# 1275468127/Medical-SAM2

Hardware: AMD Instinct MI355X
Metric: slices/sec @1024^2 (Hiera-S) (higher is better)
Workload: dtype bf16; 1 GPU; configs[1]: sam2_hiera_s 2D (train_2d SAM2 sub-sequence, forward), b=4 x 1024x1024 per GPU, 16-entry memory bank with 4 sampled memories per slice, one click per slice; forward_image -> memory_attention -> prompt encoder -> mask decoder -> memory encoder; hip_graph=True, weights=random name-keyed init

## Files before the change

### include/msam2_hip.h

```cpp
#ifndef MSAM2_HIP_H
#define MSAM2_HIP_H

#include <stddef.h>
#include <stdint.h>

#ifdef __cplusplus
extern "C" {
#endif

const char* msam2_last_error(void);

int msam2_version(void);

int msam2_operand_is_fp16(void);

int msam2_graph_begin(void* stream);

int msam2_graph_end(void* stream, void** graph_exec_out);

int msam2_graph_launch(void* graph_exec, void* stream);

int msam2_graph_destroy(void* graph_exec);

int msam2_event_create(void** ev);

int msam2_event_record(void* ev, void* stream);

int msam2_event_elapsed_ms(void* start, void* stop, float* ms);

int msam2_event_destroy(void* ev);

int msam2_gemm_nt(const void* A, int64_t lda, const void* B, int64_t ldb, const float* bias, const void* residual, int64_t ldr, void* C, int64_t ldc, int out_is_16bit, int64_t M, int64_t N, int64_t K, void* stream);

int msam2_gemm(const void* A, int64_t lda, const void* W, int64_t ldw, const float* bias, const float* colscale, const void* residual, int64_t ldr, int res_is_16bit, int64_t res_mod, void* C, int64_t ldc, int out_is_16bit, int64_t M, int64_t N, int64_t K, int act, void* stream);

int msam2_gemm_tokens(const float* A, int64_t lda, const float* A2, int64_t add_cols, const void* W, int64_t ldw, const float* bias, const float* residual, int64_t ldr, void* C, int64_t ldc, int out_is_16bit, int64_t M, int64_t N, int64_t K, int act, void* stream);

int msam2_gemm_pool2x2(const void* A, int64_t lda, const void* W, int64_t ldw, const float* bias, float* C, int64_t ldc, int64_t B, int64_t H, int64_t Wimg, int64_t N, int64_t K, void* stream);

int msam2_gemm_qkv_pool2x2(const void* A, int64_t lda, const void* W, int64_t ldw, const float* bias, void* QKV, int64_t ldc, void* Q2, int64_t ldq, int64_t B, int64_t H, int64_t Wimg, int64_t N, int64_t K, int64_t q_cols, void* stream);

int msam2_gemm_rope(const void* A, int64_t lda, const void* W, int64_t ldw, const float* bias, void* C, int64_t ldc, int64_t M, int64_t N, int64_t K, const float* rope_cos, const float* rope_sin, int64_t rope_cols, int64_t head_dim, int64_t rows_per_batch, int64_t n_rope, int64_t n_pos, void* stream);

int msam2_gemm_residual_layernorm_supported(int64_t N, int64_t K);

int msam2_gemm_residual_layernorm(const void* A, int64_t lda, const void* W, int64_t ldw, const float* bias, const float* R32, int64_t ldr, float* C32, int64_t ldc, const float* ln_w, const float* ln_b, float eps, void* Y16, int64_t ldy, int64_t M, int64_t N, int64_t K, void* stream);

int msam2_gemm_merged_residual_layernorm_supported(int64_t N, int64_t D, int splits);

int msam2_gemm_merged_residual_layernorm(const void* workspace, size_t workspace_bytes, int splits, int64_t D, const void* W, int64_t ldw, const float* bias, const float* R32, int64_t ldr, float* C32, int64_t ldc, const float* ln_w, const float* ln_b, float eps, void* Y16, int64_t ldy, int64_t M, int64_t N, void* stream);

size_t msam2_attention_workspace_bytes(int64_t Bz, int64_t H, int64_t Lq, int64_t D, int splits);

int msam2_attention_merge(void* o, const int64_t* o_strides, int64_t B, int64_t H, int64_t Lq, int64_t Lk, int64_t D, int splits, void* workspace, size_t workspace_bytes, void* stream);

int msam2_attention_fwd(const void* q, const int64_t* q_strides, const void* k, const int64_t* k_strides, const void* v, const int64_t* v_strides, void* o, const int64_t* o_strides, int64_t B, int64_t H, int64_t Lq, int64_t Lk, int64_t D, float scale, int splits, void* workspace, size_t workspace_bytes, void* stream);

int msam2_attention_fwd_lse(const void* q, const int64_t* q_strides, const void* k, const int64_t* k_strides, const void* v, const int64_t* v_strides, void* o, const int64_t* o_strides, int64_t B, int64_t H, int64_t Lq, int64_t Lk, int64_t D, float scale, int splits, void* workspace, size_t workspace_bytes, float* lse, void* stream);

int msam2_attention_fwd_lse_dropout(const void* q, const int64_t* q_strides, const void* k, const int64_t* k_strides, const void* v, const int64_t* v_strides, void* o, const int64_t* o_strides, int64_t B, int64_t H, int64_t Lq, int64_t Lk, int64_t D, float scale, int splits, void* workspace, size_t workspace_bytes, float* lse, float p, uint64_t seed, uint64_t offset, const void* seed_dev, void* stream);

int msam2_attention_kv64_fwd(const void* q, const int64_t* q_strides, const void* k, const int64_t* k_strides, const void* v, const int64_t* v_strides, void* o, const int64_t* o_strides, int64_t B, int64_t H, int64_t Lq, int64_t Lk, float scale, int splits, void* workspace, size_t workspace_bytes, void* stream);

int msam2_attention_effective_splits(int64_t Lk, int splits);

int msam2_attention_kv64_partial(const void* q, const int64_t* q_strides, const void* k, const int64_t* k_strides, const void* v, const int64_t* v_strides, int64_t B, int64_t H, int64_t Lq, int64_t Lk, float scale, int splits, int split_begin, int split_count, void* workspace, size_t workspace_bytes, void* stream);

int msam2_attention_kv64_dyn_fwd(const void* q, const int64_t* q_strides, const void* k, const int64_t* k_strides, const void* v, const int64_t* v_strides, void* o, const int64_t* o_strides, int64_t B, int64_t H, int64_t Lq, int64_t Lk, const void* key_count_dev, float scale, int splits, void* workspace, size_t workspace_bytes, void* stream);

int msam2_attention_kv64_dyn_partial(const void* q, const int64_t* q_strides, const void* k, const int64_t* k_strides, const void* v, const int64_t* v_strides, int64_t B, int64_t H, int64_t Lq, int64_t Lk, const void* key_count_dev, float scale, int splits, int split_begin, int split_count, void* workspace, size_t workspace_bytes, void* stream);

int msam2_window_attention_fwd(const void* q, int64_t q_token_stride, int64_t q_head_stride, int64_t hq, int64_t wq, int64_t ws_q, const void* k, const void* v, int64_t kv_token_stride, int64_t kv_head_stride, int64_t hk, int64_t wk, int64_t ws_k, const float* kpad, const float* vpad, void* o, int64_t o_token_stride, int64_t o_head_stride, int64_t B, int64_t H, int64_t D, float scale, void* stream);

int msam2_attention_small_fwd(const void* q, int64_t q_bs, int64_t q_ts, const void* k, int64_t k_bs, int64_t k_ts, const void* v, int64_t v_bs, int64_t v_ts, void* o, int64_t o_bs, int64_t o_ts, int64_t B, int64_t H, int64_t Lq, int64_t Lk, int64_t D, float scale, void* stream);

int msam2_attention_fewq_keysplit_splits(int64_t B, int64_t H);

int msam2_attention_fewq_keysplit(const void* q, int64_t q_bs, int64_t q_ts, const void* k, int64_t k_bs, int64_t k_ts, const void* v, int64_t v_bs, int64_t v_ts, float* part, int64_t B, int64_t H, int64_t Lq, int64_t Lk, int64_t D, int64_t splits, float scale, void* stream);

int msam2_window_qkv_attention_supported(int64_t dim, int64_t dim_out, int64_t heads, int64_t ws, int pool, int64_t H, int64_t W);

int msam2_window_qkv_attention_fwd(const void* xn, const void* w, const float* bias, void* o, int64_t B, int64_t H, int64_t W, int64_t dim, int64_t heads, int64_t ws, int pool, float scale, void* stream);

// ... 241 lines not shown
```

### medical-sam2_amd/_lib.py

```python
from __future__ import annotations

import ctypes
import os
import subprocess

_HERE = os.path.dirname(os.path.abspath(__file__))
LIB_PATH = os.environ.get("MSAM2_LIB_PATH") or os.path.join(_HERE, "libmsam2_hip.so")

c_p = ctypes.c_void_p
c_i = ctypes.c_int
c_l = ctypes.c_int64
c_f = ctypes.c_float
c_z = ctypes.c_size_t
c_d = ctypes.c_double

SIGNATURES = {
    "msam2_version": (c_i, []),
    "msam2_last_error": (ctypes.c_char_p, []),
    "msam2_operand_is_fp16": (c_i, []),
    "msam2_gemm": (c_i, [c_p, c_l, c_p, c_l, c_p, c_p, c_p, c_l, c_i, c_l, c_p, c_l, c_i, c_l, c_l, c_l, c_i, c_p]),
    "msam2_gemm_pool2x2": (c_i, [c_p, c_l, c_p, c_l, c_p, c_p, c_l, c_l, c_l, c_l, c_l, c_l, c_p]),
    "msam2_gemm_qkv_pool2x2": (c_i, [c_p, c_l, c_p, c_l, c_p, c_p, c_l, c_p, c_l, c_l, c_l, c_l, c_l, c_l, c_l, c_p]),
    "msam2_gemm_tokens": (c_i, [c_p, c_l, c_p, c_l, c_p, c_l, c_p, c_p, c_l, c_p, c_l, c_i, c_l, c_l, c_l, c_i, c_p]),
    "msam2_gemm_rope": (c_i, [c_p, c_l, c_p, c_l, c_p, c_p, c_l, c_l, c_l, c_l, c_p, c_p, c_l, c_l, c_l, c_l, c_l, c_p]),
    "msam2_gemm_residual_layernorm_supported": (c_i, [c_l, c_l]),
    "msam2_gemm_residual_layernorm": (c_i, [c_p, c_l, c_p, c_l, c_p, c_p, c_l, c_p, c_l, c_p, c_p, c_f, c_p, c_l, c_l, c_l, c_l, c_p]),
    "msam2_gemm_merged_residual_layernorm_supported": (c_i, [c_l, c_l, c_i]),
    "msam2_gemm_merged_residual_layernorm": (c_i, [c_p, c_z, c_i, c_l, c_p, c_l, c_p, c_p, c_l, c_p, c_l, c_p, c_p, c_f, c_p, c_l, c_l, c_l, c_p]),
    "msam2_ln_mlp_residual_supported": (c_i, [c_l]),
    "msam2_mlp_fused_permute_w2": (c_i, [c_p, c_p, c_l, c_l, c_p]),
    "msam2_ln_mlp_residual_fwd": (c_i, [c_p, c_l, c_l, c_p, c_p, c_f, c_p, c_p, c_p, c_p, c_p, c_p]),
    "msam2_ln_mlp_residual_fwd_dual": (c_i, [c_p, c_l, c_l, c_p, c_p, c_f, c_p, c_p, c_p, c_p, c_p, c_p, c_p]),
    "msam2_proj_ln_mlp_residual_supported": (c_i, [c_l]),
    "msam2_mlp_fused_permute_w1": (c_i, [c_p, c_p, c_l, c_l, c_p]),
    "msam2_proj_ln_mlp_residual_fwd": (c_i, [c_p, c_p, c_p, c_p, c_l, c_l, c_p, c_p, c_f, c_p, c_p, c_p, c_p, c_p, c_p, c_p, c_p, c_f, c_p, c_p]),
    "msam2_layernorm": (c_i, [c_p, c_i, c_l, c_p, c_p, c_p, c_i, c_l, c_l, c_l, c_f, c_i, c_p]),
    "msam2_layernorm_dual": (c_i, [c_p, c_l, c_p, c_p, c_p, c_l, c_p, c_l, c_l, c_l, c_f, c_p]),
    "msam2_attention_workspace_bytes": (c_z, [c_l, c_l, c_l, c_l, c_i]),
    "msam2_attention_fwd": (c_i, [c_p, c_p, c_p, c_p, c_p, c_p, c_p, c_p, c_l, c_l, c_l, c_l, c_l, c_f, c_i, c_p, c_z, c_p]),
    "msam2_attention_fwd_lse": (c_i, [c_p, c_p, c_p, c_p, c_p, c_p, c_p, c_p, c_l, c_l, c_l, c_l, c_l, c_f, c_i, c_p, c_z, c_p, c_p]),
    "msam2_attention_fwd_lse_dropout": (c_i, [c_p, c_p, c_p, c_p, c_p, c_p, c_p, c_p, c_l, c_l, c_l, c_l, c_l, c_f, c_i, c_p, c_z, c_p, c_f,
                                              ctypes.c_uint64, ctypes.c_uint64, c_p, c_p]),
    "msam2_attention_kv64_fwd": (c_i, [c_p, c_p, c_p, c_p, c_p, c_p, c_p, c_p, c_l, c_l, c_l, c_l, c_f, c_i, c_p, c_z, c_p]),
    "msam2_attention_kv64_partial": (c_i, [c_p, c_p, c_p, c_p, c_p, c_p, c_l, c_l, c_l, c_l, c_f, c_i, c_i, c_i, c_p, c_z, c_p]),
    "msam2_attention_kv64_dyn_fwd": (c_i, [c_p, c_p, c_p, c_p, c_p, c_p, c_p, c_p, c_l, c_l, c_l, c_l, c_p, c_f, c_i, c_p, c_z, c_p]),
    "msam2_attention_kv64_dyn_partial": (c_i, [c_p, c_p, c_p, c_p, c_p, c_p, c_l, c_l, c_l, c_l, c_p, c_f, c_i, c_i, c_i, c_p, c_z, c_p]),
    "msam2_attention_effective_splits": (c_i, [c_l, c_i]),
    "msam2_attention_merge": (c_i, [c_p, c_p, c_l, c_l, c_l, c_l, c_l, c_i, c_p, c_z, c_p]),
    "msam2_window_attention_fwd": (c_i, [c_p, c_l, c_l, c_l, c_l, c_l, c_p, c_p, c_l, c_l, c_l, c_l, c_l, c_p, c_p, c_p, c_l, c_l,
                                         c_l, c_l, c_l, c_f, c_p]),
    "msam2_window_qkv_attention_supported": (c_i, [c_l, c_l, c_l, c_l, c_i, c_l, c_l]),
    "msam2_window_qkv_attention_fwd": (c_i, [c_p, c_p, c_p, c_p, c_l, c_l, c_l, c_l, c_l, c_l, c_i, c_f, c_p]),
    "msam2_attention_small_fwd": (c_i, [c_p, c_l, c_l, c_p, c_l, c_l, c_p, c_l, c_l, c_p, c_l, c_l, c_l, c_l, c_l, c_l, c_l, c_f,
                                        c_p]),
    "msam2_add_cast": (c_i, [c_p, c_i, c_l, c_l, c_p, c_i, c_l, c_l, c_f, c_p, c_i, c_l, c_l, c_l, c_p]),
    "msam2_maxpool2x2": (c_i, [c_p, c_i, c_l, c_p, c_i, c_l, c_l, c_l, c_l, c_l, c_p]),
    "msam2_upsample2x_add": (c_i, [c_p, c_p, c_l, c_l, c_l, c_l, c_p]),
    "msam2_rope_table": (c_i, [c_p, c_p, c_l, c_l, c_f, c_p]),
    "msam2_rope_inplace": (c_i, [c_p, c_l, c_l, c_l, c_l, c_l, c_l, c_l, c_p, c_p, c_p]),
    "msam2_bilinear_upsample": (c_i, [c_p, c_p, c_l, c_l, c_l, c_l, c_l, c_p]),
    "msam2_sine_pos_2d": (c_i, [c_p, c_l, c_l, c_l, c_f, c_p]),
# ... 154 lines not shown
```

### medical-sam2_amd/modeling/encoder.py

```python
from __future__ import annotations

from typing import List, Optional, Tuple

import torch
import torch.nn as nn

from .. import ops
from .common import OP16, F32, WeightCache, nchw_view, to_bf16, tokens_of, v_f32, w_bf16
from .position import PositionEmbeddingSine


import os as _os
_POOL_GEMM = _os.environ.get("MSAM2_NO_POOL_GEMM") is None
_QPOOL_GEMM = _os.environ.get("MSAM2_NO_QPOOL_GEMM") is None
_FUSED_MLP = _os.environ.get("MSAM2_NO_FUSED_MLP") is None
_FUSED_QKV_ATTN = _os.environ.get("MSAM2_NO_FUSED_QKV_ATTN") is None
_FUSED_PATCH = _os.environ.get("MSAM2_NO_FUSED_PATCH") is None
_FUSED_GEMM_LN = _os.environ.get("MSAM2_NO_FUSED_GEMM_LN") is None
_FUSED_GEMM_LN_K = frozenset(int(k) for k in _os.environ.get("MSAM2_FUSED_GEMM_LN_K", "384,1536").split(",") if k.strip())
_FUSED_PROJ_MLP = _os.environ.get("MSAM2_NO_FUSED_PROJ_MLP") is None
_FUSED_PROJ_MLP_DIMS = frozenset(int(k) for k in _os.environ.get("MSAM2_FUSED_PROJ_MLP_DIMS", "96,192").split(",") if k.strip())
_FUSED_PROJ_MLP_NEXT_LN_DIMS = frozenset(int(k) for k in _os.environ.get("MSAM2_FUSED_PROJ_MLP_NEXT_LN_DIMS", "").split(",") if k.strip())
_TWO_LAUNCH = 0


class two_launch_qkv_attention:

    def __enter__(self):
        global _TWO_LAUNCH
        _TWO_LAUNCH += 1

    def __exit__(self, *exc):
        global _TWO_LAUNCH
        _TWO_LAUNCH -= 1
        return False


def _gemm_ln_dispatched(N: int, K: int) -> bool:
    return _FUSED_GEMM_LN and K in _FUSED_GEMM_LN_K and ops.gemm_residual_layernorm_supported(N, K)


def _proj_mlp_dispatched(dim_out: int, width: int) -> bool:
    return _FUSED_PROJ_MLP and width == dim_out and dim_out in _FUSED_PROJ_MLP_DIMS and ops.proj_ln_mlp_residual_supported(dim_out)


def frozen_forward_image(model, imgs: torch.Tensor) -> dict:
    with two_launch_qkv_attention():
        return model.forward_image(imgs)


class PatchEmbed(nn.Module):

    def __init__(self, kernel_size=(7, 7), stride=(4, 4), padding=(3, 3), in_chans: int = 3, embed_dim: int = 768):
        super().__init__()
        assert tuple(kernel_size) == (7, 7) and tuple(stride) == (4, 4) and tuple(padding) == (3, 3) and in_chans == 3, \
            "the HIP path implements the 7x7/4/3 RGB patch embedding used by every SAM2 config"
        self.proj = nn.Conv2d(in_chans, embed_dim, kernel_size=kernel_size, stride=stride, padding=padding)
        self._wc = WeightCache()

    def _weight(self):
        def build():
            w = torch.zeros(self.proj.weight.shape[0], 160, dtype=OP16, device=self.proj.weight.device)
            w[:, :147] = self.proj.weight.detach().reshape(-1, 147).to(OP16)
            return w
        return self._wc.get("w", [self.proj.weight], build)

    def _weight_perm(self):
        def build():
            w = self.proj.weight.detach()
            E = w.shape[0]
            wp = torch.zeros((E + 31) // 32 * 32, 22, 8, dtype=OP16, device=w.device)
            wp[:E, :21, 1:] = w.reshape(E, 21, 7).to(OP16)
            return wp.reshape(-1, 176).contiguous()
        return self._wc.get("wp", [self.proj.weight], build)

    def tokens(self, x: torch.Tensor, pos: Optional[torch.Tensor] = None) -> torch.Tensor:
        x = x.to(F32).contiguous()
        E = self.proj.weight.shape[0]
        if _FUSED_PATCH and ops.patch_embed_supported(x.shape[-1], E) and x.shape[-1] == x.shape[-2] and (pos is None or pos.shape[0] == (x.shape[-1] // 4) ** 2):
            return ops.patch_embed(x, self._weight_perm(), v_f32(self._wc, "b", self.proj.bias), None if pos is None else pos.to(F32).contiguous())
        cols = ops.im2col_patch(x)
        return ops.gemm(cols, self._weight(), v_f32(self._wc, "b", self.proj.bias), residual=pos,
                        res_mod=pos.shape[0] if pos is not None else 0, out_dtype=F32)

    def forward(self, x: torch.Tensor) -> torch.Tensor:
        B, _, S, _ = x.shape
        return self.tokens(x).reshape(B, S // 4, S // 4, -1)


class MLP(nn.Module):

    def __init__(self, input_dim: int, hidden_dim: int, output_dim: int, num_layers: int, activation: nn.Module = nn.ReLU,
                 sigmoid_output: bool = False):
        super().__init__()
        self.num_layers = num_layers
        h = [hidden_dim] * (num_layers - 1)
        self.layers = nn.ModuleList(nn.Linear(n, k) for n, k in zip([input_dim] + h, h + [output_dim]))
        self.sigmoid_output = sigmoid_output
        self.act = activation()
        self._act_code = ops.ACT_GELU if isinstance(self.act, nn.GELU) else ops.ACT_RELU
        self._wc = WeightCache()

    def run(self, x_bf16: torch.Tensor, residual: Optional[torch.Tensor] = None, out_dtype=F32, ln=None):
        h = x_bf16
        for i, layer in enumerate(self.layers):
            last = i == self.num_layers - 1
            last_act = ops.ACT_SIGMOID if self.sigmoid_output else ops.ACT_NONE
            if (last and ln is not None and residual is not None and out_dtype == F32 and last_act == ops.ACT_NONE
                    and _gemm_ln_dispatched(layer.out_features, layer.in_features)):
                return ops.gemm_residual_layernorm(h, w_bf16(self._wc, f"w{i}", layer.weight), v_f32(self._wc, f"b{i}", layer.bias), residual, *ln)
            h = ops.gemm(h, w_bf16(self._wc, f"w{i}", layer.weight), v_f32(self._wc, f"b{i}", layer.bias),
                         act=last_act if last else self._act_code, residual=residual if last else None,
                         out_dtype=out_dtype if last else OP16)
        return h if ln is None else (h, None)

    def run_tokens(self, x: torch.Tensor) -> torch.Tensor:
        L = self.layers
        if (self.num_layers == 3 and self._act_code == ops.ACT_RELU and x.shape[0] <= 4096 and L[0].in_features == 256
                and L[0].out_features == 256 and L[1].out_features == 256 and L[2].out_features <= 256):
            def pack():
                dev = x.device
                n = L[2].out_features
                w3 = torch.zeros(1, 256, 256, dtype=OP16, device=dev)
                b3 = torch.zeros(1, 256, dtype=F32, device=dev)
                w3[0, :n] = L[2].weight.detach().to(OP16)
                b3[0, :n] = L[2].bias.detach().float()
                return (L[0].weight.detach().to(OP16)[None].contiguous(), L[0].bias.detach().float()[None].contiguous(),
                        L[1].weight.detach().to(OP16)[None].contiguous(), L[1].bias.detach().float()[None].contiguous(), w3, b3)

            def consts():
                dev = x.device
                return (torch.zeros(1, dtype=torch.int32, device=dev), torch.tensor([L[2].out_features], dtype=torch.int32, device=dev),
                        torch.tensor([int(self.sigmoid_output)], dtype=torch.int32, device=dev))
            tok, od, sg = self._wc.get("tok3_const", [], consts)
            w1, b1, w2, b2, w3, b3 = self._wc.get("tok3", [t for l in L for t in (l.weight, l.bias)], pack)
            y = ops.token_mlp3(x.to(F32).contiguous().view(x.shape[0], 1, 256), tok, w1, b1, w2, b2, w3, b3, od, sg)
            return y[:, 0, : L[2].out_features].contiguous()
# ... 98 lines not shown
                q = (qp.view(B, Hq * Wq, heads, Dp) if pool else v5[:, :, 0]).permute(0, 2, 1, 3)
                o = ops.attention(q, v5[:, :, 1].permute(0, 2, 1, 3), v5[:, :, 2].permute(0, 2, 1, 3), scale=scale)
                o = o.permute(0, 2, 1, 3).reshape(B * Hq * Wq, width)
        mlp = self.mlp
        one_kernel_mlp = (_FUSED_MLP and ops.ln_mlp_residual_supported(dim_out) and mlp.num_layers == 2 and mlp._act_code == ops.ACT_GELU
                          and mlp.layers[0].out_features == 4 * dim_out and Hq * Wq >= 1024)
        if fused_gemm_ln and attn_in_one_kernel and one_kernel_mlp and _proj_mlp_dispatched(dim_out, width):
            w1p = mlp._wc.get("w0p", [mlp.layers[0].weight], lambda: ops.mlp_fused_permute_w1(mlp.layers[0].weight.detach().to(OP16).contiguous()))
            w2p = mlp._wc.get("w1p", [mlp.layers[1].weight], lambda: ops.mlp_fused_permute_w2(mlp.layers[1].weight.detach().to(OP16).contiguous()))
            next_ln = next_norm if next_norm is not None and dim_out in _FUSED_PROJ_MLP_NEXT_LN_DIMS else None
            t, out16, self.next_xn = ops.proj_ln_mlp_residual(o, proj_w, v_f32(wc, "ob", a.proj.bias), shortcut, v_f32(wc, "n2w", self.norm2.weight),
                                                              v_f32(wc, "n2b", self.norm2.bias), 1e-6, w1p, v_f32(mlp._wc, "b0", mlp.layers[0].bias),
                                                              w2p, v_f32(mlp._wc, "b1", mlp.layers[1].bias), also16=emit16, next_ln=next_ln)
            if emit16:
                self.out16 = out16
            return t, Hq, Wq
        xn2 = None
        if fused_gemm_ln and not one_kernel_mlp and _gemm_ln_dispatched(dim_out, width):
            t, xn2 = ops.gemm_residual_layernorm(o, proj_w, v_f32(wc, "ob", a.proj.bias), shortcut,
                                                 v_f32(wc, "n2w", self.norm2.weight), v_f32(wc, "n2b", self.norm2.bias), 1e-6)
        else:
            t = ops.gemm(o, proj_w, v_f32(wc, "ob", a.proj.bias), residual=shortcut, out_dtype=F32)
        if one_kernel_mlp:
            w2p = mlp._wc.get("w1p", [mlp.layers[1].weight], lambda: ops.mlp_fused_permute_w2(mlp.layers[1].weight.detach().to(OP16).contiguous()))
            t = ops.ln_mlp_residual(t, v_f32(wc, "n2w", self.norm2.weight), v_f32(wc, "n2b", self.norm2.bias), 1e-6,
                                    w_bf16(mlp._wc, "w0", mlp.layers[0].weight), v_f32(mlp._wc, "b0", mlp.layers[0].bias), w2p,
                                    v_f32(mlp._wc, "b1", mlp.layers[1].bias), also16=emit16)
            if emit16:
                t, self.out16 = t
            return t, Hq, Wq
        if xn2 is None:
            xn2 = ops.layernorm(t, v_f32(wc, "n2w", self.norm2.weight), v_f32(wc, "n2b", self.norm2.bias), 1e-6)
        if fused_gemm_ln and next_norm is not None:
            t, self.next_xn = mlp.run(xn2, residual=t, out_dtype=F32, ln=next_norm)
        else:
            t = mlp.run(xn2, residual=t, out_dtype=F32)
        return t, Hq, Wq

    def forward(self, x: torch.Tensor) -> torch.Tensor:
        B, H, W, C = x.shape
        t, h, w = self.run(x.to(F32).reshape(B * H * W, C).contiguous(), B, H, W)
        return t.reshape(B, h, w, -1)


class Hiera(nn.Module):

    def __init__(self, embed_dim: int = 96, num_heads: int = 1, drop_path_rate: float = 0.0, q_pool: int = 3,
                 q_stride: Tuple[int, int] = (2, 2), stages: Tuple[int, ...] = (2, 3, 16, 3), dim_mul: float = 2.0,
                 head_mul: float = 2.0, window_pos_embed_bkg_spatial_size: Tuple[int, int] = (14, 14),
                 window_spec: Tuple[int, ...] = (8, 4, 14, 7), global_att_blocks: Tuple[int, ...] = (12, 16, 20),
                 return_interm_layers=True):
        super().__init__()
        assert len(stages) == len(window_spec) and drop_path_rate == 0.0
        self.window_spec = window_spec
        depth = sum(stages)
        self.q_stride = q_stride
        self.stage_ends = [sum(stages[:i]) - 1 for i in range(1, len(stages) + 1)]
        self.q_pool_blocks = [x + 1 for x in self.stage_ends[:-1]][:q_pool]
        self.return_interm_layers = return_interm_layers
        self.patch_embed = PatchEmbed(embed_dim=embed_dim)
        self.global_att_blocks = global_att_blocks
        self.window_pos_embed_bkg_spatial_size = window_pos_embed_bkg_spatial_size
        self.pos_embed = nn.Parameter(torch.zeros(1, embed_dim, *window_pos_embed_bkg_spatial_size))
        self.pos_embed_window = nn.Parameter(torch.zeros(1, embed_dim, window_spec[0], window_spec[0]))
        cur_stage = 1
        self.blocks = nn.ModuleList()
        for i in range(depth):
# ... 111 lines not shown
```

### medical-sam2_amd/ops.py

```python
from __future__ import annotations

import ctypes
import math
from typing import Optional, Tuple

import torch

from ._lib import check, lib

OP16 = torch.float16 if lib().msam2_operand_is_fp16() else torch.bfloat16

F32 = torch.float32
ACT_NONE, ACT_GELU, ACT_RELU, ACT_SIGMOID = 0, 1, 2, 3


def _stream() -> int:
    return torch.cuda.current_stream().cuda_stream


def _p(t: Optional[torch.Tensor]):
    return None if t is None else t.data_ptr()


def _is_bf16(t: torch.Tensor) -> int:
# ... 195 lines not shown
    x2 = x.reshape(-1, C)
    _req(x2.dtype == F32 and x2.stride(1) == 1 and C % 4 == 0, "layernorm_dual: fp32 rows, C % 4 == 0")
    y = torch.empty(x2.shape, dtype=F32, device=x.device)
    y16 = torch.empty(x2.shape, dtype=OP16, device=x.device)
    check(lib().msam2_layernorm_dual(_p(x2), x2.stride(0), _p(weight), _p(bias), _p(y), y.stride(0), _p(y16), y16.stride(0), x2.shape[0], C, eps,
                                     _stream()))
    return y.reshape(x.shape), y16.reshape(x.shape)


def gemm_residual_layernorm_supported(N: int, K: int) -> bool:
    return bool(lib().msam2_gemm_residual_layernorm_supported(N, K))


def gemm_residual_layernorm(a: torch.Tensor, w: torch.Tensor, bias: Optional[torch.Tensor], residual: torch.Tensor, ln_w: torch.Tensor,
                            ln_b: torch.Tensor, eps: float, *, out: Optional[torch.Tensor] = None, out16: Optional[torch.Tensor] = None):
    _req(a.dim() == 2 and w.dim() == 2 and a.shape[1] == w.shape[1], f"gemm_residual_layernorm shapes {tuple(a.shape)} x {tuple(w.shape)}")
    _req(a.dtype == OP16 and w.dtype == OP16 and a.stride(1) == 1 and w.stride(1) == 1, "gemm_residual_layernorm operands: 16-bit, K-contiguous")
    M, K = a.shape
    N = w.shape[0]
    _req(gemm_residual_layernorm_supported(N, K),
         f"gemm_residual_layernorm: N = {N}, K = {K} is not built (N = 384 with K % 64 == 0; N = 256 with K = 64, 256 or 2048)")
    _req(residual.dtype == F32 and residual.shape == (M, N) and residual.stride(1) == 1, "gemm_residual_layernorm: residual must be fp32 [M, N]")
    _req(ln_w.dtype == F32 and ln_b.dtype == F32 and ln_w.numel() == N and ln_b.numel() == N and ln_w.is_contiguous() and ln_b.is_contiguous()
         and (bias is None or (bias.dtype == F32 and bias.numel() == N and bias.is_contiguous())),
         "gemm_residual_layernorm: bias, ln_w, ln_b are fp32 [N]")
    if out is None:
        out = torch.empty(M, N, dtype=F32, device=a.device)
    if out16 is None:
        out16 = torch.empty(M, N, dtype=OP16, device=a.device)
    _req(out.dtype == F32 and out.shape == (M, N) and out.stride(1) == 1 and out16.dtype == OP16 and out16.shape == (M, N) and out16.stride(1) == 1,
         "gemm_residual_layernorm: out is fp32 [M, N], out16 16-bit [M, N], rows contiguous")
    check(lib().msam2_gemm_residual_layernorm(_p(a), a.stride(0), _p(w), w.stride(0), _p(bias), _p(residual), residual.stride(0), _p(out),
                                              out.stride(0), _p(ln_w), _p(ln_b), float(eps), _p(out16), out16.stride(0), M, N, K, _stream()))
    return out, out16


def gemm_merged_residual_layernorm_supported(N: int, D: int, splits: int) -> bool:
    return bool(lib().msam2_gemm_merged_residual_layernorm_supported(N, D, splits))


def gemm_merged_residual_layernorm(workspace: torch.Tensor, splits: int, D: int, w: torch.Tensor, bias: Optional[torch.Tensor],
                                   residual: torch.Tensor, ln_w: torch.Tensor, ln_b: torch.Tensor, eps: float, *,
                                   out: Optional[torch.Tensor] = None, out16: Optional[torch.Tensor] = None):
    _req(w.dim() == 2 and w.dtype == OP16 and w.stride(1) == 1 and w.shape[1] == D, f"gemm_merged_residual_layernorm: w is 16-bit [N, {D}], K-contiguous")
    _req(workspace.dtype == torch.uint8 and workspace.is_contiguous(), "gemm_merged_residual_layernorm: workspace is a contiguous uint8 buffer")
    N = w.shape[0]
    _req(residual.dim() == 2 and residual.dtype == F32 and residual.shape[1] == N and residual.stride(1) == 1,
         "gemm_merged_residual_layernorm: residual must be fp32 [M, N]")
    M = residual.shape[0]
    _req(ln_w.dtype == F32 and ln_b.dtype == F32 and ln_w.numel() == N and ln_b.numel() == N and ln_w.is_contiguous() and ln_b.is_contiguous()
         and (bias is None or (bias.dtype == F32 and bias.numel() == N and bias.is_contiguous())),
         "gemm_merged_residual_layernorm: bias, ln_w, ln_b are fp32 [N]")
    if out is None:
        out = torch.empty(M, N, dtype=F32, device=w.device)
    if out16 is None:
        out16 = torch.empty(M, N, dtype=OP16, device=w.device)
    _req(out.dtype == F32 and out.shape == (M, N) and out.stride(1) == 1 and out16.dtype == OP16 and out16.shape == (M, N) and out16.stride(1) == 1,
         "gemm_merged_residual_layernorm: out is fp32 [M, N], out16 16-bit [M, N], rows contiguous")
    check(lib().msam2_gemm_merged_residual_layernorm(_p(workspace), workspace.numel(), int(splits), int(D), _p(w), w.stride(0), _p(bias), _p(residual),
                                                     residual.stride(0), _p(out), out.stride(0), _p(ln_w), _p(ln_b), float(eps), _p(out16),
                                                     out16.stride(0), M, N, _stream()))
    return out, out16


def ln_mlp_residual_supported(dim: int) -> bool:
    return bool(lib().msam2_ln_mlp_residual_supported(dim))
# ... 1259 lines not shown
```

Measured before the change: 754.9 slices/s.

## Fuse Hiera MLP fc1+GELU+fc2+residual+LayerNorm into one kernel for dim 384

Adds a single HIP kernel that, for each 64-row tile, computes fc1 in 128-wide hidden chunks, applies bias and GELU, keeps the hidden chunk in LDS, and accumulates fc2. It then adds the residual and writes fp32 output plus the next block's LayerNorm output. The encoder dispatches to it for 384-wide stages with at least 1024 tokens. This avoids writing the 4x-wide hidden activation to global memory and saves launches. In exchange it uses 160KB of LDS with one block per CU, and every hidden chunk runs behind serialized barriers, so the kernel may be less efficient than separate tuned GEMMs.

```diff
diff --git a/include/msam2_hip.h b/include/msam2_hip.h
--- a/include/msam2_hip.h
+++ b/include/msam2_hip.h
@@ -49,6 +49,10 @@
 int msam2_gemm_merged_residual_layernorm_supported(int64_t N, int64_t D, int splits);
 
 int msam2_gemm_merged_residual_layernorm(const void* workspace, size_t workspace_bytes, int splits, int64_t D, const void* W, int64_t ldw, const float* bias, const float* R32, int64_t ldr, float* C32, int64_t ldc, const float* ln_w, const float* ln_b, float eps, void* Y16, int64_t ldy, int64_t M, int64_t N, void* stream);
+
+int msam2_mlp_residual_layernorm_supported(int64_t N, int64_t H);
+
+int msam2_mlp_residual_layernorm_fwd(const void* A, int64_t lda, const void* W1, int64_t ldw1, const float* b1, const void* W2, int64_t ldw2, const float* b2, const float* R32, int64_t ldr, float* C32, int64_t ldc, const float* ln_w, const float* ln_b, float eps, void* Y16, int64_t ldy, int64_t M, int64_t N, int64_t H, void* stream);
 
 size_t msam2_attention_workspace_bytes(int64_t Bz, int64_t H, int64_t Lq, int64_t D, int splits);
 
diff --git a/medical-sam2_amd/_lib.py b/medical-sam2_amd/_lib.py
--- a/medical-sam2_amd/_lib.py
+++ b/medical-sam2_amd/_lib.py
@@ -27,6 +27,8 @@
     "msam2_gemm_residual_layernorm": (c_i, [c_p, c_l, c_p, c_l, c_p, c_p, c_l, c_p, c_l, c_p, c_p, c_f, c_p, c_l, c_l, c_l, c_l, c_p]),
     "msam2_gemm_merged_residual_layernorm_supported": (c_i, [c_l, c_l, c_i]),
     "msam2_gemm_merged_residual_layernorm": (c_i, [c_p, c_z, c_i, c_l, c_p, c_l, c_p, c_p, c_l, c_p, c_l, c_p, c_p, c_f, c_p, c_l, c_l, c_l, c_p]),
+    "msam2_mlp_residual_layernorm_supported": (c_i, [c_l, c_l]),
+    "msam2_mlp_residual_layernorm_fwd": (c_i, [c_p, c_l, c_p, c_l, c_p, c_p, c_l, c_p, c_p, c_l, c_p, c_l, c_p, c_p, c_f, c_p, c_l, c_l, c_l, c_l, c_p]),
     "msam2_ln_mlp_residual_supported": (c_i, [c_l]),
     "msam2_mlp_fused_permute_w2": (c_i, [c_p, c_p, c_l, c_l, c_p]),
     "msam2_ln_mlp_residual_fwd": (c_i, [c_p, c_l, c_l, c_p, c_p, c_f, c_p, c_p, c_p, c_p, c_p, c_p]),
diff --git a/medical-sam2_amd/csrc/mlp_rowln.hip b/medical-sam2_amd/csrc/mlp_rowln.hip
--- /dev/null
+++ b/medical-sam2_amd/csrc/mlp_rowln.hip
@@ -0,0 +1,344 @@
+#include "common.h"
+
+struct MlpRowLnParams {
+  const op16* A;
+  const op16* W1;
+  const op16* W2;
+  const float* b1;
+  const float* b2;
+  const float* R;
+  float* C;
+  const float* ln_w;
+  const float* ln_b;
+  op16* Y;
+  int64_t lda, ldw1, ldw2, ldr, ldc, ldy;
+  int M, H;
+  float eps;
+};
+
+template <int N, int LAD>
+__global__ __launch_bounds__(512, 1) void mlp_rowln_kernel(MlpRowLnParams p) {
+#if defined(__HIP_DEVICE_COMPILE__)
+  typedef Img128 Img;
+  constexpr int BM = 64, BK = 64, KS = BK / 16, HC = 128;
+  constexpr int KT = N / BK;
+  constexpr int A_BYTES = BM * BK * 2;
+  constexpr int RES_BYTES = KT * A_BYTES;
+  constexpr int HID_BYTES = (HC / BK) * A_BYTES;
+  constexpr int STAGE_BYTES = N * BK * 2;
+  constexpr int W1IMG_BYTES = HC * BK * 2;
+  constexpr int PPW = STAGE_BYTES / 1024 / 8;
+  constexpr int FN = N / 4 / 32;
+  constexpr int TLD = N + 4;
+  constexpr int CH = N / 64;
+  static_assert(N == 384, "one instance: the stage of 48 KB holds W1's 128 rows x 192 k as well as W2's 384 rows x 64 k");
+  static_assert((KT / 2) * W1IMG_BYTES == STAGE_BYTES && PPW * 8 * 1024 == STAGE_BYTES && BM == 8 * Img::PIECE_ROWS, "8 waves share the pieces evenly");
+  static_assert(BM * TLD * 4 <= RES_BYTES + HID_BYTES + 2 * STAGE_BYTES, "the epilogue tile aliases the images and the ring");
+  extern __shared__ __attribute__((aligned(1024))) unsigned char lds[];
+  unsigned char* const hid = lds + RES_BYTES;
+  unsigned char* const ring = hid + HID_BYTES;
+  const int tid = threadIdx.x;
+  const int wave = __builtin_amdgcn_readfirstlane(tid >> 6), lane = tid & 63;
+  const int ws = wave >> 2, wq = wave & 3;
+  const int r = lane & 31, h = lane >> 5;
+  const int64_t m0 = (int64_t)xcd_tile_order(blockIdx.x, gridDim.x) * BM;
+  if (m0 >= p.M) return;
+
+  float bias_j[FN];
+#pragma unroll
+  for (int j = 0; j < FN; ++j) bias_j[j] = p.b2 ? p.b2[wq * (N / 4) + j * 32 + r] : 0.f;
+
+  const auto a_rsrc = raw_rsrc(p.A);
+  const auto w1_rsrc = raw_rsrc(p.W1);
+  const auto w2_rsrc = raw_rsrc(p.W2);
+  unsigned offsW1[PPW], offsW2[PPW];
+#pragma unroll
+  for (int i = 0; i < PPW; ++i) {
+    const int q = wave * PPW + i;
+    const int row1 = Img::piece_row(q & 15, lane);
+    offsW1[i] = (unsigned)((int64_t)row1 * p.ldw1 * 2 + (q >> 4) * (BK * 2) + Img::src_chunk(row1, lane) * 16);
+    const int row2 = Img::piece_row(q, lane);
+    offsW2[i] = (unsigned)((int64_t)row2 * p.ldw2 * 2 + Img::src_chunk(row2, lane) * 16);
+  }
+  auto issue = [&](int c, int t) __attribute__((always_inline)) {
+    unsigned char* base = ring + (t & 1) * STAGE_BYTES + wave * (PPW * 1024);
+    if ((LAD & 8) && c > 0) return;
+    if (t < 2) {
+      const unsigned so = (unsigned)((int64_t)c * HC * p.ldw1 * 2) + (unsigned)t * (N / 2) * 2;
+#pragma unroll
+      for (int i = 0; i < PPW; ++i) glds16(w1_rsrc, base + i * 1024, offsW1[i], so);
+    } else {
+      const unsigned so = (unsigned)(c * HC + (t - 2) * BK) * 2;
+#pragma unroll
+      for (int i = 0; i < PPW; ++i) glds16(w2_rsrc, base + i * 1024, offsW2[i], so);
+    }
+  };
+
+  {
+    const int row = Img::piece_row(wave, lane);
+    const unsigned offsA = (unsigned)(min(m0 + row, (int64_t)p.M - 1) * p.lda * 2 + Img::src_chunk(row, lane) * 16);
+#pragma unroll
+    for (int i = 0; i < KT; ++i) glds16(a_rsrc, lds + i * A_BYTES + wave * 1024, offsA, (unsigned)i * BK * 2);
+  }
+  {
+    const int j = (blockIdx.x >> 3) & 31;
+    unsigned char* dst = ring + STAGE_BYTES + wave * 1024;
+    {
+      const int cpr = N >> 3, rows = p.H >> 5, n = rows * cpr;
+      for (int i = wave; i * 64 < n; i += 8) {
+        const int q = min(i * 64 + lane, n - 1);
+        const int row = j * rows + q / cpr, c = q - (q / cpr) * cpr;
+        glds16(w1_rsrc, dst, (unsigned)((int64_t)row * p.ldw1 * 2 + c * 16), 0);
+      }
+    }
+    {
+      const int cpr = p.H >> 3, n = (N / 32) * cpr;
+      for (int i = wave; i * 64 < n; i += 8) {
+        const int q = min(i * 64 + lane, n - 1);
+        const int row = j * (N / 32) + q / cpr, c = q - (q / cpr) * cpr;
+        glds16(w2_rsrc, dst, (unsigned)((int64_t)row * p.ldw2 * 2 + c * 16), 0);
+      }
+    }
+  }
+
+  f32x16 acc[FN];
+  zero_acc(acc);
+
+  const int ra = ws * 32 + r;
+  const int offA = ra * Img::ROW_BYTES, swzA = Img::swz(ra);
+  const int r1 = wq * 32 + r;
+  const int offW1 = r1 * Img::ROW_BYTES, swzW1 = Img::swz(r1);
+  int offB[FN], swzB[FN];
+#pragma unroll
+  for (int j = 0; j < FN; ++j) {
+    const int rb = wq * (N / 4) + j * 32 + r;
+    offB[j] = rb * Img::ROW_BYTES;
+    swzB[j] = Img::swz(rb);
+  }
+  unsigned char* const hdst = hid + (wq >> 1) * A_BYTES + offA + 8 * h;
+  const int hc0 = (wq & 1) * 4;
+
+  f32x16 acc1;
+  f32x4 b1v[4];
+  auto fc1_half = [&](int t) __attribute__((always_inline)) {
+    const unsigned char* sb = ring + (t & 1) * STAGE_BYTES;
+#pragma unroll
+    for (int kl = 0; kl < KT / 2; ++kl) {
+      const unsigned char* sw = sb + kl * W1IMG_BYTES;
+      const unsigned char* sx = lds + (t * (KT / 2) + kl) * A_BYTES;
+      op16x8 wf[KS], xf[KS];
+#pragma unroll
+      for (int ks = 0; ks < KS; ++ks) {
+        const int c = 2 * ks + h;
+        wf[ks] = *reinterpret_cast<const op16x8*>(sw + offW1 + ((c ^ swzW1) << 4));
+        xf[ks] = *reinterpret_cast<const op16x8*>(sx + offA + ((c ^ swzA) << 4));
+      }
+#pragma unroll
+      for (int ks = 0; ks < KS; ++ks) {
+        if constexpr (LAD & 2) acc1[ks] += op2f(wf[ks][0]) + op2f(xf[ks][0]);
+        else acc1 = MSAM2_MFMA_32x32x16(wf[ks], xf[ks], acc1, 0, 0, 0);
+      }
+    }
+  };
+  auto fc2_step = [&](int u) __attribute__((always_inline)) {
+    const unsigned char* sb = ring + u * STAGE_BYTES;
+    const unsigned char* sa = hid + u * A_BYTES;
+    op16x8 af[KS], bfr[KS][FN];
+#pragma unroll
+    for (int ks = 0; ks < KS; ++ks) {
+      const int c = 2 * ks + h;
+      af[ks] = *reinterpret_cast<const op16x8*>(sa + offA + ((c ^ swzA) << 4));
+#pragma unroll
+      for (int j = 0; j < FN; ++j) bfr[ks][j] = *reinterpret_cast<const op16x8*>(sb + offB[j] + ((c ^ swzB[j]) << 4));
+    }
+#pragma unroll
+    for (int ks = 0; ks < KS; ++ks)
+#pragma unroll
+      for (int j = 0; j < FN; ++j) {
+        if constexpr (LAD & 4) acc[j][ks] += op2f(af[ks][0]) + op2f(bfr[ks][j][0]);
+        else acc[j] = MSAM2_MFMA_32x32x16(af[ks], bfr[ks][j], acc[j], 0, 0, 0);
+      }
+  };
+
+  const int nc = p.H / HC;
+  issue(0, 0);
+  for (int c = 0; c < nc; ++c) {
+    wait_vmcnt<0>();
+    __builtin_amdgcn_s_barrier();
+    issue(c, 1);
+#pragma unroll
+    for (int g = 0; g < 4; ++g)
+      b1v[g] = p.b1 ? *reinterpret_cast<const f32x4*>(p.b1 + c * HC + wq * 32 + 8 * g + 4 * h) : f32x4{0.f, 0.f, 0.f, 0.f};
+#pragma unroll
+    for (int e = 0; e < 16; ++e) acc1[e] = 0.f;
+    fc1_half(0);
+    wait_vmcnt<0>();
+    __builtin_amdgcn_s_barrier();
+    issue(c, 2);
+    fc1_half(1);
+#pragma unroll
+    for (int g = 0; g < 4; ++g) {
+      f32x2 g0 = f32x2{acc1[4 * g] + b1v[g][0], acc1[4 * g + 1] + b1v[g][1]};
+      f32x2 g1 = f32x2{acc1[4 * g + 2] + b1v[g][2], acc1[4 * g + 3] + b1v[g][3]};
+      if constexpr (!(LAD & 1)) {
+        g0 = gelu_erf2(g0);
+        g1 = gelu_erf2(g1);
+      }
+      op16x4 o;
+      o[0] = f2op(g0[0]);
+      o[1] = f2op(g0[1]);
+      o[2] = f2op(g1[0]);
+      o[3] = f2op(g1[1]);
+      *reinterpret_cast<op16x4*>(hdst + (((hc0 + g) ^ swzA) << 4)) = o;
+    }
+    __builtin_amdgcn_fence(__ATOMIC_RELEASE, "workgroup");
+    wait_vmcnt<0>();
+    __builtin_amdgcn_s_barrier();
+    issue(c, 3);
+    fc2_step(0);
+    wait_vmcnt<0>();
+    __builtin_amdgcn_s_barrier();
+    if (c + 1 < nc) issue(c + 1, 0);
+    fc2_step(1);
+  }
+  wait_vmcnt<0>();
+  __builtin_amdgcn_s_barrier();
+
+  const int l16 = lane & 15;
+  int64_t grow[2];
+  f32x4 rv[2][CH], ww[CH], bb[CH];
+#pragma unroll
+  for (int ps = 0; ps < 2; ++ps) {
+    grow[ps] = m0 + ps * 32 + wave * 4 + (lane >> 4);
+    const float* rr = p.R + min(grow[ps], (int64_t)p.M - 1) * p.ldr;
+#pragma unroll
+    for (int j = 0; j < CH; ++j) rv[ps][j] = *reinterpret_cast<const f32x4*>(rr + (l16 + 16 * j) * 4);
+  }
+#pragma unroll
+  for (int j = 0; j < CH; ++j) {
+    ww[j] = *reinterpret_cast<const f32x4*>(p.ln_w + (l16 + 16 * j) * 4);
+    bb[j] = *reinterpret_cast<const f32x4*>(p.ln_b + (l16 + 16 * j) * 4);
+  }
+  float* tile = reinterpret_cast<float*>(lds);
+#pragma unroll
+  for (int j = 0; j < FN; ++j)
+#pragma unroll
+    for (int e = 0; e < 16; ++e)
+      tile[(ws * 32 + s_frag_key(e, h)) * TLD + wq * (N / 4) + j * 32 + r] = acc[j][e] + bias_j[j];
+  __builtin_amdgcn_s_barrier();
+  float v[2][CH][4];
+#pragma unroll
+  for (int ps = 0; ps < 2; ++ps) {
+    const float* trow = tile + (ps * 32 + wave * 4 + (lane >> 4)) * TLD;
+#pragma unroll
+    for (int j = 0; j < CH; ++j) {
+      const f32x4 t = *reinterpret_cast<const f32x4*>(trow + (l16 + 16 * j) * 4);
+#pragma unroll
+      for (int e = 0; e < 4; ++e) v[ps][j][e] = t[e] + rv[ps][j][e];
+    }
+  }
+#pragma unroll
+  for (int ps = 0; ps < 2; ++ps) {
+    if (grow[ps] < p.M) {
+      float* cr = p.C + grow[ps] * p.ldc;
+#pragma unroll
+      for (int j = 0; j < CH; ++j) *reinterpret_cast<f32x4*>(cr + (l16 + 16 * j) * 4) = f32x4{v[ps][j][0], v[ps][j][1], v[ps][j][2], v[ps][j][3]};
+    }
+  }
+  if (!p.Y) return;
+#pragma unroll
+  for (int ps = 0; ps < 2; ++ps) {
+    float s = 0.f;
+#pragma unroll
+    for (int j = 0; j < CH; ++j)
+#pragma unroll
+      for (int e = 0; e < 4; ++e) s += v[ps][j][e];
+    group16_add(s);
+    const float mean = s / N;
+    float q = 0.f;
+#pragma unroll
+    for (int j = 0; j < CH; ++j)
+#pragma unroll
+      for (int e = 0; e < 4; ++e) {
+        const float d = v[ps][j][e] - mean;
+        q += d * d;
+      }
+    group16_add(q);
+    const float rstd = 1.0f / sqrtf(q / N + p.eps);
+    if (grow[ps] < p.M) {
+      op16* yr = p.Y + grow[ps] * p.ldy;
+#pragma unroll
+      for (int j = 0; j < CH; ++j) {
+        op16x4 o;
+#pragma unroll
+        for (int e = 0; e < 4; ++e) {
+          const float u = (v[ps][j][e] - mean) * rstd * ww[j][e] + bb[j][e];
+          o[e] = f2out<op16>(u);
+        }
+        *reinterpret_cast<op16x4*>(yr + (l16 + 16 * j) * 4) = o;
+      }
+    }
+  }
+#endif
+}
+
+template <int LAD>
+static int launch_mlp_rowln(const MlpRowLnParams& p, void* stream) {
+  constexpr int LDS = 160 * 1024;
+  ensure_dyn_lds<mlp_rowln_kernel<384, LAD>>(LDS);
+  hipLaunchKernelGGL((mlp_rowln_kernel<384, LAD>), dim3(cdiv(p.M, 64)), dim3(512), LDS, (hipStream_t)stream, p);
+  return msam2_check_launch("mlp_residual_layernorm");
+}
+
+extern "C" int msam2_mlp_residual_layernorm_supported(int64_t N, int64_t H) { return (N == 384 && H > 0 && H % 128 == 0) ? 1 : 0; }
+
+extern "C" int msam2_mlp_residual_layernorm_fwd(const void* A, int64_t lda, const void* W1, int64_t ldw1, const float* b1, const void* W2,
+                                                int64_t ldw2, const float* b2, const float* R32, int64_t ldr, float* C32, int64_t ldc,
+                                                const float* ln_w, const float* ln_b, float eps, void* Y16, int64_t ldy, int64_t M, int64_t N,
+                                                int64_t H, void* stream) {
+  MSAM2_REQUIRE(A && W1 && W2 && R32 && C32, "mlp_residual_layernorm: null operand");
+  MSAM2_REQUIRE(!Y16 || (ln_w && ln_b), "mlp_residual_layernorm: LayerNorm rows asked for without ln_w, ln_b");
+  MSAM2_REQUIRE(msam2_mlp_residual_layernorm_supported(N, H), "mlp_residual_layernorm: N=%lld H=%lld is not built (N = 384 with H %% 128 == 0)",
+                (long long)N, (long long)H);
+  MSAM2_REQUIRE(M > 0 && M < (1ll << 31) - 64, "mlp_residual_layernorm: M=%lld", (long long)M);
+  MSAM2_REQUIRE(lda % 8 == 0 && ldw1 % 8 == 0 && ldw2 % 8 == 0 && lda >= N && ldw1 >= N && ldw2 >= H,
+                "mlp_residual_layernorm: lda, ldw1, ldw2 must be multiples of 8 (16-byte rows), lda, ldw1 >= N, ldw2 >= H");
+  MSAM2_REQUIRE(ldr % 4 == 0 && ldc % 4 == 0 && ldr >= N && ldc >= N && (!Y16 || (ldy % 4 == 0 && ldy >= N)),
+                "mlp_residual_layernorm: ldr, ldc, ldy must be multiples of 4, >= N");
+  MSAM2_REQUIRE(vec_ok(8, 2, A, W1, W2) &&
+                    vec_ok(4, 4, (const void*)b1, (const void*)b2, (const void*)R32, (const void*)C32, (const void*)ln_w, (const void*)ln_b) &&
+                    vec_ok(4, 2, (const void*)Y16),
+                "mlp_residual_layernorm: A, W1, W2, b1, b2, R32, C32, ln_w, ln_b must be 16-byte aligned, Y16 8-byte");
+  MSAM2_REQUIRE(M * lda * 2 < (1ll << 31) && H * ldw1 * 2 < (1ll << 31) && N * ldw2 * 2 < (1ll << 31),
+                "mlp_residual_layernorm: A / W1 / W2 beyond the 2 GB of a buffer descriptor's offsets");
+  MlpRowLnParams p = {};
+  p.A = (const op16*)A; p.W1 = (const op16*)W1; p.W2 = (const op16*)W2; p.b1 = b1; p.b2 = b2; p.R = R32; p.C = C32;
+  p.ln_w = Y16 ? ln_w : (const float*)R32; p.ln_b = Y16 ? ln_b : (const float*)R32;
+  p.Y = (op16*)Y16;
+  p.lda = lda; p.ldw1 = ldw1; p.ldw2 = ldw2; p.ldr = ldr; p.ldc = ldc; p.ldy = ldy;
+  p.M = (int)M; p.H = (int)H; p.eps = eps;
+  return launch_mlp_rowln<0>(p, stream);
+}
+
+#ifdef MSAM2_MLP_ROWLN_LADDER
+extern "C" {
+int msam2_mlp_rowln_ladder(int lad, const void* A, const void* W1, const void* W2, const float* R32, float* C32, const float* ln_w,
+                                      const float* ln_b, void* Y16, int64_t M, int64_t H, void* stream) {
+  MSAM2_REQUIRE(A && W1 && W2 && R32 && C32 && ln_w && ln_b && Y16 && M > 0 && H > 0 && H % 128 == 0, "mlp_rowln_ladder: operands");
+  MlpRowLnParams p = {};
+  p.A = (const op16*)A; p.W1 = (const op16*)W1; p.W2 = (const op16*)W2; p.R = R32; p.C = C32; p.ln_w = ln_w; p.ln_b = ln_b; p.Y = (op16*)Y16;
+  p.lda = 384; p.ldw1 = 384; p.ldw2 = H; p.ldr = 384; p.ldc = 384; p.ldy = 384;
+  p.M = (int)M; p.H = (int)H; p.eps = 1e-6f;
+  switch (lad) {
+    case 0: return launch_mlp_rowln<0>(p, stream);
+    case 1: return launch_mlp_rowln<1>(p, stream);
+    case 2: return launch_mlp_rowln<3>(p, stream);
+    case 3: return launch_mlp_rowln<4>(p, stream);
+    case 4: return launch_mlp_rowln<7>(p, stream);
+    case 5: return launch_mlp_rowln<15>(p, stream);
+    case 6: return launch_mlp_rowln<8>(p, stream);
+    default: MSAM2_REQUIRE(false, "mlp_rowln_ladder: variant %d", lad);
+  }
+}
+}
+#endif
diff --git a/medical-sam2_amd/modeling/encoder.py b/medical-sam2_amd/modeling/encoder.py
--- a/medical-sam2_amd/modeling/encoder.py
+++ b/medical-sam2_amd/modeling/encoder.py
@@ -18,6 +18,8 @@
 _FUSED_PATCH = _os.environ.get("MSAM2_NO_FUSED_PATCH") is None
 _FUSED_GEMM_LN = _os.environ.get("MSAM2_NO_FUSED_GEMM_LN") is None
 _FUSED_GEMM_LN_K = frozenset(int(k) for k in _os.environ.get("MSAM2_FUSED_GEMM_LN_K", "384,1536").split(",") if k.strip())
+_FUSED_MLP_LN = _os.environ.get("MSAM2_NO_FUSED_MLP_LN") is None
+_FUSED_MLP_LN_MIN_TOKENS = 1024
 _FUSED_PROJ_MLP = _os.environ.get("MSAM2_NO_FUSED_PROJ_MLP") is None
 _FUSED_PROJ_MLP_DIMS = frozenset(int(k) for k in _os.environ.get("MSAM2_FUSED_PROJ_MLP_DIMS", "96,192").split(",") if k.strip())
 _FUSED_PROJ_MLP_NEXT_LN_DIMS = frozenset(int(k) for k in _os.environ.get("MSAM2_FUSED_PROJ_MLP_NEXT_LN_DIMS", "").split(",") if k.strip())
@@ -38,6 +40,10 @@
 
 def _gemm_ln_dispatched(N: int, K: int) -> bool:
     return _FUSED_GEMM_LN and K in _FUSED_GEMM_LN_K and ops.gemm_residual_layernorm_supported(N, K)
+
+
+def _mlp_ln_dispatched(N: int, H: int) -> bool:
+    return _FUSED_GEMM_LN and _FUSED_MLP_LN and ops.mlp_residual_layernorm_supported(N, H)
 
 
 def _proj_mlp_dispatched(dim_out: int, width: int) -> bool:
@@ -101,8 +107,14 @@
         self._act_code = ops.ACT_GELU if isinstance(self.act, nn.GELU) else ops.ACT_RELU
         self._wc = WeightCache()
 
-    def run(self, x_bf16: torch.Tensor, residual: Optional[torch.Tensor] = None, out_dtype=F32, ln=None):
+    def run(self, x_bf16: torch.Tensor, residual: Optional[torch.Tensor] = None, out_dtype=F32, ln=None, one_kernel: bool = False):
         h = x_bf16
+        if (one_kernel and ln is not None and residual is not None and out_dtype == F32 and self.num_layers == 2 and not self.sigmoid_output
+                and self._act_code == ops.ACT_GELU and _mlp_ln_dispatched(self.layers[1].out_features, self.layers[0].out_features)
+                and self.layers[0].in_features == self.layers[1].out_features):
+            l0, l1 = self.layers
+            return ops.mlp_residual_layernorm(h, w_bf16(self._wc, "w0", l0.weight), v_f32(self._wc, "b0", l0.bias),
+                                              w_bf16(self._wc, "w1", l1.weight), v_f32(self._wc, "b1", l1.bias), residual, *ln)
         for i, layer in enumerate(self.layers):
             last = i == self.num_layers - 1
             last_act = ops.ACT_SIGMOID if self.sigmoid_output else ops.ACT_NONE
@@ -267,7 +279,7 @@
         if xn2 is None:
             xn2 = ops.layernorm(t, v_f32(wc, "n2w", self.norm2.weight), v_f32(wc, "n2b", self.norm2.bias), 1e-6)
         if fused_gemm_ln and next_norm is not None:
-            t, self.next_xn = mlp.run(xn2, residual=t, out_dtype=F32, ln=next_norm)
+            t, self.next_xn = mlp.run(xn2, residual=t, out_dtype=F32, ln=next_norm, one_kernel=Hq * Wq >= _FUSED_MLP_LN_MIN_TOKENS)
         else:
             t = mlp.run(xn2, residual=t, out_dtype=F32)
         return t, Hq, Wq
diff --git a/medical-sam2_amd/ops.py b/medical-sam2_amd/ops.py
--- a/medical-sam2_amd/ops.py
+++ b/medical-sam2_amd/ops.py
@@ -251,6 +251,37 @@
          "gemm_residual_layernorm: out is fp32 [M, N], out16 16-bit [M, N], rows contiguous")
     check(lib().msam2_gemm_residual_layernorm(_p(a), a.stride(0), _p(w), w.stride(0), _p(bias), _p(residual), residual.stride(0), _p(out),
                                               out.stride(0), _p(ln_w), _p(ln_b), float(eps), _p(out16), out16.stride(0), M, N, K, _stream()))
+    return out, out16
+
+
+def mlp_residual_layernorm_supported(N: int, H: int) -> bool:
+    return bool(lib().msam2_mlp_residual_layernorm_supported(N, H))
+
+
+def mlp_residual_layernorm(a: torch.Tensor, w1: torch.Tensor, b1: Optional[torch.Tensor], w2: torch.Tensor, b2: Optional[torch.Tensor],
+                           residual: torch.Tensor, ln_w: torch.Tensor, ln_b: torch.Tensor, eps: float, *, out: Optional[torch.Tensor] = None,
+                           out16: Optional[torch.Tensor] = None):
+    _req(a.dim() == 2 and w1.dim() == 2 and w2.dim() == 2 and a.shape[1] == w1.shape[1] and w2.shape == (w1.shape[1], w1.shape[0]),
+         f"mlp_residual_layernorm shapes {tuple(a.shape)} x {tuple(w1.shape)} x {tuple(w2.shape)}")
+    _req(a.dtype == OP16 and w1.dtype == OP16 and w2.dtype == OP16 and a.stride(1) == 1 and w1.stride(1) == 1 and w2.stride(1) == 1,
+         "mlp_residual_layernorm operands: 16-bit, reduction dimension contiguous")
+    M, N = a.shape
+    H = w1.shape[0]
+    _req(mlp_residual_layernorm_supported(N, H), f"mlp_residual_layernorm: N = {N}, H = {H} is not built (N = 384 with H % 128 == 0)")
+    _req(residual.dtype == F32 and residual.shape == (M, N) and residual.stride(1) == 1, "mlp_residual_layernorm: residual must be fp32 [M, N]")
+    _req(ln_w.dtype == F32 and ln_b.dtype == F32 and ln_w.numel() == N and ln_b.numel() == N and ln_w.is_contiguous() and ln_b.is_contiguous()
+         and (b1 is None or (b1.dtype == F32 and b1.numel() == H and b1.is_contiguous()))
+         and (b2 is None or (b2.dtype == F32 and b2.numel() == N and b2.is_contiguous())),
+         "mlp_residual_layernorm: b1 is fp32 [H]; b2, ln_w, ln_b are fp32 [N]")
+    if out is None:
+        out = torch.empty(M, N, dtype=F32, device=a.device)
+    if out16 is None:
+        out16 = torch.empty(M, N, dtype=OP16, device=a.device)
+    _req(out.dtype == F32 and out.shape == (M, N) and out.stride(1) == 1 and out16.dtype == OP16 and out16.shape == (M, N) and out16.stride(1) == 1,
+         "mlp_residual_layernorm: out is fp32 [M, N], out16 16-bit [M, N], rows contiguous")
+    check(lib().msam2_mlp_residual_layernorm_fwd(_p(a), a.stride(0), _p(w1), w1.stride(0), _p(b1), _p(w2), w2.stride(0), _p(b2), _p(residual),
+                                                 residual.stride(0), _p(out), out.stride(0), _p(ln_w), _p(ln_b), float(eps), _p(out16),
+                                                 out16.stride(0), M, N, H, _stream()))
     return out, out16
 
 
```

After: 785.6 slices/s (median of 6 runs). 1.04x the previous value.
